# PreferredAI/PyBMF

Hardware: AMD Instinct MI355X
Metric: MU iterations/sec (BinaryMF-Penalty, 100k x 20k Boolean, k=64) (higher is better)
Workload: dtype i8 (bits x int8 digit planes on the integer MFMA, exact int32 accumulation); fp64 master factors and scalars; 1 GPU; BinaryMF-Penalty MU, 100000x20000 dense Boolean X, k=64, reg=1 growth=1.02, init normal+balance seed 2024; mae_pass=False, operands=i8x3, splits_xv=2, splits_xtu=11

## Files before the change

### include/bmf_hip.h

```cpp
#ifndef BMF_HIP_H
#define BMF_HIP_H

#include <stdint.h>

#ifdef __cplusplus
extern "C" {
#endif

#define BMF_OK 0
#define BMF_ERR_BAD_ARG (-1)
#define BMF_ERR_HIP (-2)
#define BMF_ERR_UNSUPPORTED (-3)
#define BMF_ERR_COMM (-4)

#define BMF_ROW_PAD 512
#define BMF_RED_PAD 128
#define BMF_MAX_KP 64
#define BMF_LOG_COLS 16

#define BMF_MODE_PREPARE 0
#define BMF_MODE_PENALTY 1
#define BMF_MODE_WNMF 2

enum {
// ... 146 lines not shown
int bmf_mae_sum_ex(const uint32_t* XTbits, int64_t ldxt, int64_t m_pad, int64_t n_pad, const float* U, const float* V, int kp,
                   uint16_t* ws, double* sum, int one_product, void* stream);
int bmf_mae_sum_tiled(const uint32_t* XTtiled, int64_t ldxt, int64_t m_pad, int64_t n_pad, const float* U, const float* V, int kp,
                      uint16_t* ws, double* sum, void* stream);

int bmf_mae_plan(int64_t m_pad, int64_t n_pad, int* groups, int* stages_per_group);


int bmf_cover_count(const uint32_t* Xbits, int64_t rows_pad, int64_t ldx, int64_t words, const uint64_t* rowbits,
                    const uint32_t* colbits, int64_t ldcb, int kp, unsigned long long* counts, const int32_t* stop,
                    void* stream);

int bmf_cover_delta(const uint32_t* bits, int64_t ld, int64_t words, int64_t rows_pad, const uint64_t* rowbits,
                    const uint64_t* rowbits_prev, const uint32_t* colbits, int64_t ldcb, int kp, unsigned long long* counts,
                    const uint64_t* copy_src, uint64_t* copy_dst, int64_t copy_n, const int32_t* stop, void* stream);

int bmf_confusion_rows(const uint32_t* Gbits, int64_t ldg, const uint32_t* Pbits, int64_t ldp, int64_t rows, int64_t words,
                       uint32_t* tp, uint32_t* fp, void* stream);

int bmf_boolean_product_bits(const uint64_t* rowbits, int64_t rows, const uint32_t* colbits, int64_t ldcb, int kp,
                             int64_t words, uint32_t* out, int64_t ldo, void* stream);

int bmf_real_product(const float* U, int64_t m_pad, int32_t m, const float* V, int64_t n_pad, int32_t n, int kp, float* out,
                     int64_t ldo, void* stream);


int bmf_residual_sums(const uint32_t* Xbits, int64_t m_pad, int64_t ldx, int32_t m, int32_t n, const float* U,
                      const float* V, int kp, double* sums, const int32_t* stop, void* stream);

int bmf_residual_plan(int64_t m, int64_t n, int* col_groups, int* tiles_per_group);
// ... 408 lines not shown
```

### pybmf_amd/_lib.py

```python
from __future__ import annotations

import ctypes as C
import os

import torch

_HERE = os.path.dirname(os.path.abspath(__file__))
LIB_PATH = os.path.join(_HERE, "csrc", os.environ.get("BMF_LIB", "libbmf_hip.so"))

BMF_OK = 0
ROW_PAD = 512
PANEL_BF16, PANEL_F16, PANEL_I8 = 0, 1, 2
LINK_SIGMOID, LINK_KL = 1, 2
PALM_ELBMF, PALM_PRIMP = 1, 2
NORM_SPECTRAL, NORM_FROBENIUS = 0, 1
RED_PAD = 128
MAX_KP = 64
LOG_COLS = 16
MODE_PREPARE, MODE_PENALTY, MODE_WNMF = 0, 1, 2
(LOG_ITER, LOG_ERROR, LOG_REC, LOG_REG, LOG_REGERR, LOG_RMSE, LOG_MAE, LOG_TP, LOG_FP, LOG_FN, LOG_TN, LOG_VALID,
 LOG_STOP) = range(13)

_vp, _i32, _i64, _f32, _f64 = C.c_void_p, C.c_int32, C.c_int64, C.c_float, C.c_double

# ... 137 lines not shown
    "bmf_mu_epilogue": (C.c_int, [C.POINTER(EpilogueArgs), _vp]),
    "bmf_masked_pass": (C.c_int, [_vp, _vp, _vp, _vp, _i32, _vp, _vp, _i32, _vp, _vp, _vp, C.c_int, _vp, _vp, _vp, _vp, _vp]),
    "bmf_masked_link_pass": (C.c_int, [_vp, _vp, _vp, _vp, _i32, _vp, _vp, _i32, _vp, _vp, _vp, C.c_int, _vp, _vp, _vp, _vp, C.c_int, _f64, _vp]),
    "bmf_masked_link_pass_k": (C.c_int, [_vp, _vp, _vp, _vp, _i32, _vp, _vp, _i32, _vp, _vp, _vp, C.c_int, C.c_int, _vp, _vp, _vp, _vp, C.c_int, _f64, _vp]),
    "bmf_masked_counts": (C.c_int, [_vp, _vp, _vp, _i64, _vp, _vp, _vp, _vp]),
    "bmf_masked_pass_wide": (C.c_int, [_vp, _vp, _vp, _vp, _i32, _vp, _vp, _i32, _vp] + [_vp] * 12),
    "bmf_masked_counts_wide": (C.c_int, [_vp, _vp, _vp, _i64, _vp, _vp, _vp, _vp, _vp, _vp]),
    "bmf_real_confusion": (C.c_int, [_vp, _i64, _i32, _i32, _vp, _vp, _vp, _vp]),
    "bmf_confusion_rows": (C.c_int, [_vp, _i64, _vp, _i64, _i64, _i64, _vp, _vp, _vp]),
    "bmf_mae_sum": (C.c_int, [_vp, _i64, _i64, _i64, _vp, _vp, C.c_int, _vp, _vp, _vp]),
    "bmf_mae_sum_ex": (C.c_int, [_vp, _i64, _i64, _i64, _vp, _vp, C.c_int, _vp, _vp, C.c_int, _vp]),
    "bmf_mae_sum_tiled": (C.c_int, [_vp, _i64, _i64, _i64, _vp, _vp, C.c_int, _vp, _vp, _vp]),
    "bmf_mae_plan": (C.c_int, [_i64, _i64, C.POINTER(C.c_int), C.POINTER(C.c_int)]),
    "bmf_cover_count": (C.c_int, [_vp, _i64, _i64, _i64, _vp, _vp, _i64, C.c_int, _vp, _vp, _vp]),
    "bmf_cover_delta": (C.c_int, [_vp, _i64, _i64, _i64, _vp, _vp, _vp, _i64, C.c_int, _vp, _vp, _vp, _i64, _vp, _vp]),
    "bmf_boolean_product_bits": (C.c_int, [_vp, _i64, _vp, _i64, C.c_int, _i64, _vp, _i64, _vp]),
    "bmf_real_product": (C.c_int, [_vp, _i64, _i32, _vp, _i64, _i32, C.c_int, _vp, _i64, _vp]),
    "bmf_residual_sums": (C.c_int, [_vp, _i64, _i64, _i32, _i32, _vp, _vp, C.c_int, _vp, _vp, _vp]),
    "bmf_residual_plan": (C.c_int, [_i64, _i64, C.POINTER(C.c_int), C.POINTER(C.c_int)]),
    "bmf_sqdiff_work": (_i64, []),
    "bmf_sqdiff_sum": (C.c_int, [_vp, _vp, _vp, _i64, _vp, _vp, _vp]),
    "bmf_residual_sums_f32": (C.c_int, [_vp, _i64, _i64, _i32, _i32, _vp, _vp, C.c_int, _vp, _vp]),
    "bmf_penalty_prepare": (C.c_int, [C.POINTER(PenaltyState), _vp]),
    "bmf_penalty_update": (C.c_int, [C.POINTER(PenaltyState), _f64, _vp]),
    "bmf_penalty_update_head": (C.c_int, [C.POINTER(PenaltyState), _f64, _vp]),
    "bmf_penalty_update_xtu": (C.c_int, [C.POINTER(PenaltyState), _i32, _vp]),
    "bmf_penalty_finalize": (C.c_int, [C.POINTER(PenaltyState), _i32, _f64, _i32, _vp]),
    "bmf_penalty_run": (C.c_int, [C.POINTER(PenaltyState), _i32, _i32, C.POINTER(_f64), _i32, _vp]),
    "bmf_comm_available": (C.c_int, []),
    "bmf_comm_unique_id": (C.c_int, [_vp]),
# ... 146 lines not shown
```

### pybmf_amd/csrc/api.hip

```cpp
#include "common.h"
#include "comm.h"

#include <cstdlib>
#include <vector>

int bmf_xf_bits_launch(const uint32_t* Abits, int64_t rows_pad, int64_t ldw, int64_t red_words, const uint16_t* panel,
                        int64_t ldp, int terms, int kp, float* out, int64_t slab_stride, int splits, int panel_kind,
                        const float* colscale, const int32_t* stop, hipStream_t s);
int bmf_mae_launch(const uint32_t* XTbits, int64_t ldxt, int64_t m_pad, int64_t n_pad, const float* U, const float* V, int kp,
                   uint16_t* ws, double* sum, const int32_t* stop, hipStream_t s, int one_product, int x_tiled, int zero_sums);
int bmf_panel_f16_launch(const float* F, int64_t rows_pad, int64_t ldf, int kp, uint16_t* panel, int64_t ldp, float* ws,
                         float* scale, bool have_blockmax, const int32_t* stop, hipStream_t s);
int bmf_panel_i8_launch(const double* F64, const float* F, int64_t rows_pad, int64_t ldf, int kp, int limbs, int8_t* panel, int64_t ldp,
                        float* ws, float* scale, bool have_blockmax, const int32_t* stop, hipStream_t s, bool have_scale,
                        const float* flags, float* colscale_out, const float* rslabs, int rcount, int rn, float* rout32, double* rout64);
int bmf_gram_partial_launch(const float* F, int64_t rows_pad, int64_t ldf, int kp, float* slabs, int blocks, const float* blockmax, int limbs,
                            float* scale, const int32_t* stop, hipStream_t s, int fused);
int bmf_xf_bits_i8_launch(const uint32_t* Abits, int64_t rows_pad, int64_t ldw, int64_t red_words, const int8_t* panel, int64_t ldp,
                          int limbs, const float* colscale, int kp, int col0, int ncols, float* out, int64_t slab_stride, int splits,
                          int a_tiled, const int32_t* stop, hipStream_t s);
int bmf_cover_launch(const uint32_t* Xbits, int64_t rows_pad, int64_t ldx, int64_t words, const uint64_t* rowbits,
                     const uint32_t* colbits, int64_t ldcb, int kp, unsigned long long* counts, const int32_t* stop,
                     hipStream_t s);
int bmf_cover_delta_launch(const uint32_t* bits, int64_t ld, int64_t words, int64_t rows_pad, const uint64_t* rowbits,
                           const uint64_t* rowbits_prev, const uint32_t* colbits, int64_t ldcb, int kp, unsigned long long* counts,
                           const uint64_t* copy_src, uint64_t* copy_dst, int64_t copy_n, const int32_t* stop, hipStream_t s);
int bmf_residual_launch(const uint32_t* Xbits, int64_t m_pad, int64_t ldx, int m, int n, const float* A, const float* B,
                        const float* dA, const float* dB, int kp, double* sums, const int32_t* stop, hipStream_t s);

namespace {
struct Timer {
    bool on = false, open = false;
    int cap = 0, used = 0, every = 1, seen = 0;
    std::vector<hipEvent_t> ev;
} g_timer;
}

void bmf_timer_begin(hipStream_t s) {
    g_timer.open = g_timer.on && g_timer.used < g_timer.cap && (g_timer.seen++ % g_timer.every) == 0;
    if (g_timer.open) (void)hipEventRecord(g_timer.ev[2 * g_timer.used], s);
}
// ... 267 lines not shown
        for (int sp = 0; sp < (stopped ? 0 : count); ++sp) acc += *reinterpret_cast<const f32x4*>(slabs + (int64_t)sp * slab_stride + row * kp + 32 * block + c4);
        *reinterpret_cast<f32x4*>(out + ((int64_t)block * rows_pad + row) * 32 + c4) = acc;
    }
}
}

static int xtu_slots_used(const bmf_penalty_state* st) {
    int n = st->splits_xtu;
    if (st->panel_kind == BMF_PANEL_I8) {
        const int need = bmf_xf_bits_i8_slots(st->n_pad, st->m_pad / 32, st->nred_blocks == 2 ? 32 : st->kp);
        if (need >= 1 && need < n) n = need;
    }
    return n;
}

enum { SWEEP_HEAD = 1, SWEEP_XTU = 2, SWEEP_SCALARS = 4, SWEEP_ALL = 7 };
static int sweep(const bmf_penalty_state* st, int mode, double reg, hipStream_t s, int phase = SWEEP_ALL, int block = -1, bool gather_in_finalize = false,
                 bool reduce_in_finalize = false) {
    const int kp = st->kp, kk = kp * kp;
    const int32_t* stop = st->stop;
    const bool f16 = st->panel_kind == BMF_PANEL_F16, i8 = st->panel_kind == BMF_PANEL_I8;
    const bool blocked = st->nred_blocks == 2;
    static const bool fused_planes = [] { const char* e = getenv("BMF_I8_FUSED_PLANES"); return !(e && e[0] == '0'); }();
    const int epi_terms = (f16 || i8) ? 0 : st->terms;
    const bool delta = st->ubits_prev && !st->updates_only;

    if (phase & SWEEP_HEAD) {
        bmf_epilogue_args ev = {};
        ev.F64 = st->V64; ev.F = st->V; ev.rows_pad = st->n_pad; ev.rows = st->n; ev.k = st->k; ev.kp = kp;
        ev.num = mode == BMF_MODE_PREPARE ? nullptr : st->Nred; ev.slab_stride = st->n_pad * kp; ev.splits = 1;
        ev.num_block_stride = blocked ? st->n_pad * 32 : 0;
        ev.G = st->GU; ev.reg = reg; ev.mode = mode; ev.thr = st->thr_v; ev.terms = epi_terms;
        ev.panel = st->Vpanel; ev.ldp = st->n_pad; ev.rowbits = st->vbits; ev.colbits = st->vcolbits; ev.ldcb = st->ldvc;
        ev.partials = st->partV; ev.stop = stop; ev.blockmax = (f16 || i8) ? st->panel_ws : nullptr;
        if (i8 && fused_planes) { ev.planes = (int8_t*)st->Vpanel; ev.plane_scale = st->scaleV; ev.limbs = st->terms; }
        BMF_TRY(bmf_mu_epilogue(&ev, s));
        if (f16) BMF_TRY(bmf_panel_f16_launch(st->V, st->n_pad, kp, kp, st->Vpanel, st->n_pad, st->panel_ws, st->scaleV, true, stop, s));
        BMF_TRY(bmf_gram_partial_launch(st->V, st->n_pad, kp, kp, st->gram_slabs, st->gram_blocks, i8 ? st->panel_ws : nullptr, st->terms, st->scaleV, stop, s, fused_planes ? 1 : 0));
        if (i8 && fused_planes)
            BMF_TRY(bmf_panel_i8_launch(st->V64, st->V, st->n_pad, kp, kp, st->terms, (int8_t*)st->Vpanel, st->n_pad, st->panel_ws, st->scaleV + 2 * kp, true, stop, s, true,
                                        st->scaleV + 3 * kp, st->scaleV + kp, st->gram_slabs, st->gram_blocks, kk, st->GV, st->GV64));
        else {
            if (i8)
                BMF_TRY(bmf_panel_i8_launch(st->V64, st->V, st->n_pad, kp, kp, st->terms, (int8_t*)st->Vpanel, st->n_pad, st->panel_ws, st->scaleV, true, stop, s, true, nullptr, nullptr,
                                            nullptr, 0, 0, nullptr, nullptr));
            BMF_TRY(bmf_reduce_slabs(st->gram_slabs, kk, st->gram_blocks, kk, st->GV, st->GV64, s));
        }
        if (delta && mode != BMF_MODE_PREPARE)
            BMF_TRY(bmf_cover_delta_launch(st->XTbits, st->ldxt, st->m_pad / 32, st->n_pad, st->vbits, st->vbits_prev, st->ucolbits, st->lduc, kp,
                                           st->counts, st->ubits, st->ubits_prev, st->m_pad, stop, s));

        bmf_timer_begin(s);
        if (i8)
            BMF_TRY(bmf_xf_bits_i8_launch(st->Xtiled ? st->Xtiled : st->Xbits, st->m_pad, st->ldx, st->n_pad / 32, (const int8_t*)st->Vpanel,
                                          st->n_pad, st->terms, st->scaleV + kp, kp, 0, kp, st->Mslab, st->m_pad * kp, st->splits_xv,
                                          st->Xtiled != nullptr, stop, s));
        else
            BMF_TRY(bmf_xf_bits_launch(st->Xbits, st->m_pad, st->ldx, st->n_pad / 32, st->Vpanel, st->n_pad, st->terms, kp, st->Mslab,
                                       st->m_pad * kp, st->splits_xv, st->panel_kind, f16 ? st->scaleV + kp : nullptr, stop, s));
        bmf_timer_end(s);

        bmf_epilogue_args eu = {};
        eu.F64 = st->U64; eu.F = st->U; eu.rows_pad = st->m_pad; eu.rows = st->m; eu.k = st->k; eu.kp = kp;
        const bool presum = st->splits_xv >= 6;
        if (presum)
            BMF_TRY(bmf_reduce_slabs(st->Mslab, st->m_pad * kp, st->splits_xv, st->m_pad * kp, st->Mslab, nullptr, s));
        eu.num = st->Mslab; eu.slab_stride = st->m_pad * kp; eu.splits = presum ? 1 : st->splits_xv;
        eu.G = st->GV; eu.reg = reg; eu.mode = mode; eu.thr = st->thr_u; eu.terms = epi_terms;
        eu.panel = st->Upanel; eu.ldp = st->m_pad; eu.rowbits = st->ubits; eu.colbits = st->ucolbits; eu.ldcb = st->lduc;
        eu.partials = st->partU; eu.stop = stop; eu.blockmax = (f16 || i8) ? st->panel_ws : nullptr;
        if (i8 && fused_planes) { eu.planes = (int8_t*)st->Upanel; eu.plane_scale = st->scaleU; eu.limbs = st->terms; }
        BMF_TRY(bmf_mu_epilogue(&eu, s));
        if (f16) BMF_TRY(bmf_panel_f16_launch(st->U, st->m_pad, kp, kp, st->Upanel, st->m_pad, st->panel_ws, st->scaleU, true, stop, s));
        BMF_TRY(bmf_gram_partial_launch(st->U, st->m_pad, kp, kp, st->gram_slabs, st->gram_blocks, i8 ? st->panel_ws : nullptr, st->terms, st->scaleU, stop, s, fused_planes ? 1 : 0));
        if (i8 && fused_planes)
            BMF_TRY(bmf_panel_i8_launch(st->U64, st->U, st->m_pad, kp, kp, st->terms, (int8_t*)st->Upanel, st->m_pad, st->panel_ws, st->scaleU + 2 * kp, true, stop, s, true,
                                        st->scaleU + 3 * kp, st->scaleU + kp, st->gram_slabs, st->gram_blocks, kk, nullptr, st->comm + 8));
        else {
            if (i8)
                BMF_TRY(bmf_panel_i8_launch(st->U64, st->U, st->m_pad, kp, kp, st->terms, (int8_t*)st->Upanel, st->m_pad, st->panel_ws, st->scaleU, true, stop, s, true, nullptr, nullptr,
                                            nullptr, 0, 0, nullptr, nullptr));
            BMF_TRY(bmf_reduce_slabs(st->gram_slabs, kk, st->gram_blocks, kk, nullptr, st->comm + 8, s));
        }
    }
    if (phase & SWEEP_SCALARS) {
        if (delta && mode != BMF_MODE_PREPARE) {
            BMF_TRY(bmf_cover_delta_launch(st->Xbits, st->ldx, st->n_pad / 32, st->m_pad, st->ubits, st->ubits_prev, st->vcolbits, st->ldvc, kp,
                                           st->counts, st->vbits, st->vbits_prev, st->n_pad, stop, s));
        } else if (!st->updates_only) {
            BMF_TRY(bmf_cover_launch(st->Xbits, st->m_pad, st->ldx, st->n_pad / 32, st->ubits, st->vcolbits, st->ldvc, kp, st->counts,
                                     stop, s));
            if (delta) {
                BMF_LAUNCH(rebase_cover_kernel, dim3(64), dim3(256), 0, s, st->ubits, st->ubits_prev, st->m_pad, st->vbits, st->vbits_prev, st->n_pad,
                           st->counts, stop);
                BMF_LAUNCH_CHECK();
            }
        }
        if (st->with_mae && !st->updates_only) {
            const bool one_product = st->m_pad * st->n_pad >= (1 << 24);
            if (!(st->mae_ws && one_product)) BMF_LAUNCH(zero_mae_kernel, dim3(1), dim3(64), 0, s, st->comm, stop);
            if (st->mae_ws) {
                const bool xt = st->XTtiled && st->m_pad * st->n_pad >= (1 << 24) && st->n_pad % 256 == 0 && st->ldxt % 16 == 0 && st->ldxt * 32 == st->m_pad;
                BMF_TRY(bmf_mae_launch(xt ? st->XTtiled : st->XTbits, st->ldxt, st->m_pad, st->n_pad, st->U, st->V, kp, st->mae_ws, st->comm + 4, stop, s,
// ... 96 lines not shown
}

static bool overlap_exchange(const bmf_penalty_state* st, const bmf_comm* c) {
    static const int env = [] { const char* e = getenv("BMF_EXCHANGE_OVERLAP"); return e ? (e[0] == '0' ? 0 : 1) : -1; }();
    if (env >= 0) return env == 1;
    if (c->world <= 1 || st->updates_only) return false;
    if (st->exchange_overlap != 0) return st->exchange_overlap == 2;
    return bmf_exchange_overlap_rule(st->with_mae, st->m_pad) != 0;
}

int exchange_phase(const bmf_penalty_state* st, bmf_comm* c, hipStream_t s) {
    const int kp = st->kp;
    const int64_t n32 = st->n_pad * kp, n64 = 8 + (int64_t)kp * kp;
    const bool timed = c->t_used < c->t_cap;
    const bool overlap = overlap_exchange(st, c);
    if (!overlap) BMF_TRY(sweep(st, st->mode, 0.0, s, SWEEP_SCALARS));
    if (timed) BMF_HIP_CHECK(hipEventRecord(c->tev[3 * c->t_used], s));
    if (st->nred_blocks == 2) {
        BMF_TRY(sweep(st, st->mode, 0.0, s, SWEEP_XTU, 0));
        BMF_TRY(fence_to_comm(c, 0, s));
        if (overlap) {
            BMF_TRY(bmf_comm_allreduce_on(c, st->Nred, n32 / 2, BMF_DTYPE_F32, c->cs));
        } else {
            BMF_TRY(bmf_comm_group_begin(c));
            int rc = bmf_comm_allreduce_on(c, st->Nred, n32 / 2, BMF_DTYPE_F32, c->cs);
            if (rc == BMF_OK) rc = bmf_comm_allreduce_on(c, st->comm, n64, BMF_DTYPE_F64, c->cs);
            const int rce = bmf_comm_group_end(c);
            if (rc != BMF_OK || rce != BMF_OK) return rc != BMF_OK ? rc : rce;
        }
        BMF_TRY(sweep(st, st->mode, 0.0, s, SWEEP_XTU, 1));
        BMF_TRY(fence_to_comm(c, 1, s));
// ... 64 lines not shown
    BMF_LAUNCH(finalize_kernel, dim3(1), dim3(1024), 0, s, *st, 0, reg0, (int)max_iter, 0);
    BMF_LAUNCH_CHECK();
    return BMF_OK;
}

extern "C" int bmf_penalty_run_sharded(const bmf_penalty_state* st, bmf_comm* comm, int32_t iter0, int32_t iter1, const double* regs_host,
                                       int32_t max_iter, void* stream) {
    BMF_TRY(check_state(st, "bmf_penalty_run_sharded"));
    BMF_TRY(check_comm(st, comm, "bmf_penalty_run_sharded"));
    BMF_REQUIRE(regs_host, "bmf_penalty_run_sharded: null regs_host");
    BMF_REQUIRE(iter0 >= 1 && iter1 >= iter0 && iter1 <= st->log_rows, "bmf_penalty_run_sharded: bad iteration range [%d,%d) for %d log rows",
                iter0, iter1, st->log_rows);
    hipStream_t s = (hipStream_t)stream;
    for (int it = iter0; it < iter1; ++it) {
        const double reg = regs_host[it - iter0];
        BMF_TRY(sweep(st, st->mode, reg, s, SWEEP_HEAD));
        BMF_TRY(exchange_phase(st, comm, s));
        BMF_LAUNCH(finalize_kernel, dim3(1), dim3(1024), 0, s, *st, it, reg, (int)max_iter, 0);
        BMF_LAUNCH_CHECK();
    }
    return BMF_OK;
}
```

### pybmf_amd/csrc/common.h

```cpp
#pragma once
#include <hip/hip_runtime.h>
#include <stdint.h>
#include <stdio.h>
#include <stdarg.h>

#include "../../include/bmf_hip.h"

typedef __attribute__((ext_vector_type(8))) __bf16 bf16x8;
typedef __attribute__((ext_vector_type(16))) float f32x16;
typedef __attribute__((ext_vector_type(4))) float f32x4;
typedef __attribute__((ext_vector_type(4))) unsigned u32x4;
typedef __attribute__((ext_vector_type(2))) unsigned u32x2;

#define BMF_EPS_F 2.220446049250313e-16f
#define BMF_EPS_D 2.220446049250313e-16

void bmf_set_error(const char* fmt, ...);
#define BMF_REQUIRE(cond, ...)                 \
    do {                                       \
        if (!(cond)) {                         \
            bmf_set_error(__VA_ARGS__);        \
            return BMF_ERR_BAD_ARG;            \
        }                                      \
    } while (0)
// ... 81 lines not shown
    }
    return t;
}
__device__ __forceinline__ double wave_sum(double v) {
#pragma unroll
    for (int o = 32; o > 0; o >>= 1) v += __shfl_xor(v, o, 64);
    return v;
}
__device__ __forceinline__ unsigned wave_sum(unsigned v) {
#pragma unroll
    for (int o = 32; o > 0; o >>= 1) v += __shfl_xor(v, o, 64);
    return v;
}

__device__ __forceinline__ void bmf_colscale_i8_block(const float* __restrict__ blockmax, int nblk, int kp, int limbs,
                                                      float* __restrict__ scale, int blk, float* sh) {
    const int cl = threadIdx.x & 3, sub = threadIdx.x >> 2;
    const int c = blk * 4 + cl;
    float m0 = 0.f;
    for (int b = sub; b < nblk; b += 64) m0 = fmaxf(m0, blockmax[(int64_t)b * kp + c]);
    sh[threadIdx.x] = m0;
    __syncthreads();
    for (int o = 128; o >= 4; o >>= 1) {
        if (threadIdx.x < o) sh[threadIdx.x] = fmaxf(sh[threadIdx.x], sh[threadIdx.x + o]);
        __syncthreads();
    }
    if (threadIdx.x < 4) {
        const float m = sh[threadIdx.x];
        int e = 0;
        if (m > 0.f && m <= 3.0e38f) {
            int ex;
            const float f = frexpf(m, &ex);
#ifdef BMF_EXP_QMAX_FRAC
            e = min(max((f > BMF_EXP_QMAX_FRAC ? BMF_EXP_QMAX_EXP - 1 : BMF_EXP_QMAX_EXP) - ex, -100), 100);
#else
            e = min(max((f > 0.99599f ? 22 : 23) - ex, -100), 100);
#endif
        }
        scale[c] = ldexpf(1.0f, e);
        scale[kp + c] = ldexpf(1.0f, (limbs == 2 ? 8 : 0) - e);
    }
}

__device__ __forceinline__ void bmf_colscale_i8_fused_block(const float* __restrict__ blockmax, int nblk, int kp, int limbs,
                                                            float* __restrict__ scale, int blk, float* sh) {
    const int cl = threadIdx.x & 3, sub = threadIdx.x >> 2;
    const int c = blk * 4 + cl;
    float m0 = 0.f;
    for (int b = sub; b < nblk; b += 64) m0 = fmaxf(m0, blockmax[(int64_t)b * kp + c]);
    sh[threadIdx.x] = m0;
    __syncthreads();
    for (int o = 128; o >= 4; o >>= 1) {
        if (threadIdx.x < o) sh[threadIdx.x] = fmaxf(sh[threadIdx.x], sh[threadIdx.x + o]);
        __syncthreads();
    }
    if (threadIdx.x < 4) {
        const float m = sh[threadIdx.x];
        int e = 0;
        if (m > 0.f && m <= 3.0e38f) {
            int ex;
            const float f = frexpf(m, &ex);
#ifdef BMF_EXP_QMAX_FRAC
            e = min(max((f > BMF_EXP_QMAX_FRAC ? BMF_EXP_QMAX_EXP - 1 : BMF_EXP_QMAX_EXP) - ex, -100), 100);
#else
            e = min(max((f > 0.99599f ? 22 : 23) - ex, -100), 100);
#endif
        }
        const float used = scale[c];
        const float v = m * used;
#ifdef BMF_EXP_QMAX_FRAC
        const bool ok = used > 0.f && used <= 3.0e38f && (m == 0.f || (v <= BMF_EXP_QMAX_FRAC * (float)(1 << BMF_EXP_QMAX_EXP) && v >= (float)(1 << (BMF_EXP_QMAX_EXP - 2))));
#else
        const bool ok = used > 0.f && used <= 3.0e38f && (m == 0.f || (v <= 8355711.0f && v >= 2097152.0f));
#endif
        const float fresh = ldexpf(1.0f, e);
        scale[kp + c] = (limbs == 2 ? 256.0f : 1.0f) / (ok ? used : fresh);
        scale[2 * kp + c] = fresh;
        scale[3 * kp + c] = ok ? 0.0f : 1.0f;
        scale[c] = fresh;
    }
}

__device__ __forceinline__ uint16_t bf16_bits(float x) {
    __bf16 b = (__bf16)x;
    return __builtin_bit_cast(uint16_t, b);
}
__device__ __forceinline__ float bf16_to_f32(uint16_t b) { return __uint_as_float(((unsigned)b) << 16); }

__device__ __forceinline__ void bmf_split3_bf16(const float (&x)[8], u32x4& hi, u32x4& mid, u32x4& lo) {
    unsigned xb[8], mb[8], lb[8];
#pragma unroll
    for (int j = 0; j < 8; ++j) {
        xb[j] = __float_as_uint(x[j]);
        const float r1 = x[j] - __uint_as_float(xb[j] & 0xffff0000u);
        mb[j] = __float_as_uint(r1);
        lb[j] = __float_as_uint(r1 - __uint_as_float(mb[j] & 0xffff0000u));
    }
// ... 11 lines not shown
```

### pybmf_amd/csrc/cover.hip

```cpp
#include "common.h"

#include <algorithm>
#include <cstdlib>

namespace {

constexpr int RB = 8, NW = 8;
constexpr int CH = 256;

__global__ __launch_bounds__(512) void cover_kernel(const uint32_t* __restrict__ X, int64_t ldx, int64_t words,
                                                     const uint64_t* __restrict__ rowbits,
                                                     const uint32_t* __restrict__ colbits, int64_t ldcb, int kp,
                                                     int64_t rows_pad, int rows_per_block, int y_big, int rows_big,
                                                     unsigned long long* __restrict__ counts,
                                                     const int32_t* __restrict__ stop) {
    if (stop && *stop != 0) return;
    __shared__ __attribute__((aligned(16))) uint32_t vt[BMF_MAX_KP + 1][CH];
    const int lane = threadIdx.x & 63;
    const int wave = __builtin_amdgcn_readfirstlane(threadIdx.x >> 6);
    const int64_t w0 = (int64_t)blockIdx.x * CH;
    const int nw = (int)min((int64_t)CH, words - w0);

    {
        constexpr int PIECES = BMF_MAX_KP * CH / 4;
// ... 224 lines not shown
    }
    tp = wave_sum(tp);
    pp = wave_sum(pp);
    __syncthreads();
    if (lane == 0) { vt[wave] = tp; vt[NWV + wave] = pp; }
    __syncthreads();
    if (threadIdx.x < 2) {
        unsigned long long t = 0, a_ = 0;
#pragma unroll
        for (int w = 0; w < NWV; ++w) { t += vt[w]; a_ += vt[NWV + w]; }
        const unsigned long long val = threadIdx.x == 0 ? t : a_ - t;
        if (val) atomicAdd(&counts[threadIdx.x], val);
    }
}

__global__ __launch_bounds__(1024) void cover_delta_kernel(const uint32_t* __restrict__ X, int64_t ldx, int64_t words, int chunk_words,
                                                            const uint64_t* __restrict__ rowbits, const uint64_t* __restrict__ rowbits_prev,
                                                            const uint32_t* __restrict__ colbits, int64_t ldcb, int kp, int64_t rows_pad,
                                                            int rows_per_block, unsigned long long* __restrict__ counts,
                                                            const uint64_t* __restrict__ copy_src, uint64_t* __restrict__ copy_dst, int64_t copy_n,
                                                            const int32_t* __restrict__ stop) {
    if (stop && *stop != 0) return;
    constexpr int CW = 640, NWV = 16, NS = 3;
    __shared__ __attribute__((aligned(16))) uint32_t vt[BMF_MAX_KP * CW];
    const int lane = threadIdx.x & 63;
    const int wave = __builtin_amdgcn_readfirstlane(threadIdx.x >> 6);
    const int64_t w0 = (int64_t)blockIdx.x * chunk_words;
    const int nw = (int)min((int64_t)chunk_words, words - w0);
    const int64_t r0 = (int64_t)blockIdx.y * rows_per_block;
    const int64_t r1 = min(r0 + rows_per_block, rows_pad);

    if (copy_n > 0) {
        const int64_t nthreads = (int64_t)gridDim.x * gridDim.y * 1024;
        for (int64_t i = ((int64_t)blockIdx.y * gridDim.x + blockIdx.x) * 1024 + threadIdx.x; i < copy_n; i += nthreads) copy_dst[i] = copy_src[i];
    }

    unsigned long long need = 0ull;
    for (int64_t r = r0 + threadIdx.x; r < r1; r += 1024) {
        const unsigned long long a_ = rowbits[r], b_ = rowbits_prev[r];
        if (a_ != b_) need |= a_ | b_;
    }
    if (threadIdx.x < 2) vt[threadIdx.x] = 0u;
    __syncthreads();
    if (need) {
        atomicOr(&vt[0], (unsigned)need);
        atomicOr(&vt[1], (unsigned)(need >> 32));
    }
    __syncthreads();
    need = ((unsigned long long)vt[1] << 32) | vt[0];
// ... 144 lines not shown
#pragma unroll
            for (int sg = 0; sg < NS; ++sg) x_cur[sg] = x_nxt[sg];
        }
    }
    int tp = (int)wave_sum(tpn - tpo);
    int pp = (int)wave_sum(ppn - ppo);
    __syncthreads();
    if (lane == 0) { vt[wave] = (unsigned)tp; vt[NWV + wave] = (unsigned)pp; }
    __syncthreads();
    if (threadIdx.x < 2) {
        long long t = 0, a_ = 0;
#pragma unroll
        for (int w = 0; w < NWV; ++w) { t += (int)vt[w]; a_ += (int)vt[NWV + w]; }
        const long long val = threadIdx.x == 0 ? t : a_ - t;
        if (val) atomicAdd(&counts[threadIdx.x], (unsigned long long)val);
    }
}

__global__ __launch_bounds__(256) void product_bits_kernel(const uint64_t* __restrict__ rowbits, int64_t rows,
                                                            const uint32_t* __restrict__ colbits, int64_t ldcb, int64_t words,
                                                            uint32_t* __restrict__ out, int64_t ldo) {
    const int64_t total = rows * words;
    for (int64_t idx = (int64_t)blockIdx.x * 256 + threadIdx.x; idx < total; idx += (int64_t)gridDim.x * 256) {
        const int64_t row = idx / words, w = idx - row * words;
        unsigned long long u = rowbits[row];
        unsigned pd = 0u;
        while (u) {
            const int l = __builtin_ctzll(u);
            u &= u - 1;
            pd |= colbits[(int64_t)l * ldcb + w];
// ... 96 lines not shown
}

extern "C" int bmf_cover_count(const uint32_t* Xbits, int64_t rows_pad, int64_t ldx, int64_t words,
                               const uint64_t* rowbits, const uint32_t* colbits, int64_t ldcb, int kp,
                               unsigned long long* counts, const int32_t* stop, void* stream) {
    BMF_REQUIRE(Xbits && rowbits && colbits && counts, "bmf_cover_count: null pointer");
    BMF_REQUIRE(rows_pad > 0 && rows_pad % 64 == 0, "bmf_cover_count: rows_pad must be a positive multiple of 64");
    BMF_REQUIRE(words > 0 && words % 4 == 0 && ldx >= words && ldx % 4 == 0, "bmf_cover_count: words/ldx must be multiples of 4, ldx >= words");
    BMF_REQUIRE(ldcb >= words && ldcb % 4 == 0, "bmf_cover_count: ldcb must be >= words and a multiple of 4");
    BMF_REQUIRE(bmf_aligned16(colbits), "bmf_cover_count: colbits must be 16-byte aligned");
    BMF_REQUIRE(kp >= 1 && kp <= BMF_MAX_KP, "bmf_cover_count: kp must be 1..64");
    BMF_REQUIRE(bmf_aligned16(Xbits), "bmf_cover_count: Xbits must be 16-byte aligned");
    return bmf_cover_launch(Xbits, rows_pad, ldx, words, rowbits, colbits, ldcb, kp, counts, stop, (hipStream_t)stream);
}

int bmf_cover_delta_launch(const uint32_t* bits, int64_t ld, int64_t words, int64_t rows_pad, const uint64_t* rowbits,
                           const uint64_t* rowbits_prev, const uint32_t* colbits, int64_t ldcb, int kp, unsigned long long* counts,
                           const uint64_t* copy_src, uint64_t* copy_dst, int64_t copy_n, const int32_t* stop, hipStream_t s) {
    const int chunks_w = (int)((words + 639) / 640);
    const int64_t per = (words + chunks_w - 1) / chunks_w;
    const int cw = (int)(words >= 128 ? (per + 127) / 128 * 128 : words);
    const int cus = bmf_cu_count_current();
    int64_t groups = cus / chunks_w > 0 ? cus / chunks_w : 1;
    const int64_t units = rows_pad / 64;
    if (groups > units) groups = units;
    const int rows_per_block = (int)(((units + groups - 1) / groups) * 64);
    groups = (rows_pad + rows_per_block - 1) / rows_per_block;
    BMF_LAUNCH(cover_delta_kernel, dim3((unsigned)chunks_w, (unsigned)groups), dim3(1024), 0, s, bits, ld, words, cw, rowbits, rowbits_prev, colbits,
               ldcb, kp, rows_pad, rows_per_block, counts, copy_src, copy_dst, copy_n, stop);
    BMF_LAUNCH_CHECK();
    return BMF_OK;
}

extern "C" int bmf_cover_delta(const uint32_t* bits, int64_t ld, int64_t words, int64_t rows_pad, const uint64_t* rowbits,
                               const uint64_t* rowbits_prev, const uint32_t* colbits, int64_t ldcb, int kp, unsigned long long* counts,
                               const uint64_t* copy_src, uint64_t* copy_dst, int64_t copy_n, const int32_t* stop, void* stream) {
    BMF_REQUIRE(bits && rowbits && rowbits_prev && colbits && counts, "bmf_cover_delta: null pointer");
    BMF_REQUIRE(rows_pad > 0 && rows_pad % 64 == 0, "bmf_cover_delta: rows_pad must be a positive multiple of 64");
    BMF_REQUIRE(words >= 4 && words % 4 == 0 && ld >= words && ld % 4 == 0, "bmf_cover_delta: words/ld must be multiples of 4, ld >= words >= 4");
    BMF_REQUIRE(ldcb >= words && ldcb % 4 == 0, "bmf_cover_delta: ldcb must be >= words and a multiple of 4");
    BMF_REQUIRE(bmf_aligned16(bits) && bmf_aligned16(colbits), "bmf_cover_delta: bits and colbits must be 16-byte aligned");
    BMF_REQUIRE(kp >= 1 && kp <= BMF_MAX_KP, "bmf_cover_delta: kp must be 1..64");
    BMF_REQUIRE(copy_n >= 0 && (copy_n == 0 || (copy_src && copy_dst)), "bmf_cover_delta: copy_n > 0 needs copy_src and copy_dst");
    BMF_REQUIRE(copy_n == 0 || (copy_dst != rowbits && copy_dst != rowbits_prev), "bmf_cover_delta: the copy must not overwrite the words this launch compares");
    return bmf_cover_delta_launch(bits, ld, words, rows_pad, rowbits, rowbits_prev, colbits, ldcb, kp, counts, copy_src, copy_dst, copy_n, stop,
                                  (hipStream_t)stream);
// ... 14 lines not shown
```

Baseline: 1941 iterations/s.

## Merge Gram partial and cover-delta kernels into one role-split launch

Adds a combined kernel in which some workgroups run the cover-delta bit counting, others compute the Gram partial slabs, and a few compute the i8 column scales, all in a single launch. The sweep uses it in place of separate Gram and cover-delta launches for the V side, and also for the U side when the scalar phase runs with the head. This moves the row cover-delta out of the scalar phase. The aim is to save launches and let the two independent workloads share the GPU at the same time. The cost is larger per-block LDS and register use and workgroups that serialize cover-delta then Gram work, which may lengthen the critical path.

```diff
diff --git a/include/bmf_hip.h b/include/bmf_hip.h
--- a/include/bmf_hip.h
+++ b/include/bmf_hip.h
@@ -184,6 +184,12 @@
 int bmf_cover_delta(const uint32_t* bits, int64_t ld, int64_t words, int64_t rows_pad, const uint64_t* rowbits,
                     const uint64_t* rowbits_prev, const uint32_t* colbits, int64_t ldcb, int kp, unsigned long long* counts,
                     const uint64_t* copy_src, uint64_t* copy_dst, int64_t copy_n, const int32_t* stop, void* stream);
+
+int bmf_gram_cover_delta(const float* F, int64_t rows_pad, int64_t ldf, int kp, float* slabs, int blocks, const float* blockmax, int limbs,
+                         float* scale, int fused, const uint32_t* bits, int64_t ld, int64_t words, int64_t bit_rows_pad,
+                         const uint64_t* rowbits, const uint64_t* rowbits_prev, const uint32_t* colbits, int64_t ldcb,
+                         unsigned long long* counts, const uint64_t* copy_src, uint64_t* copy_dst, int64_t copy_n, const int32_t* stop,
+                         void* stream);
 
 int bmf_confusion_rows(const uint32_t* Gbits, int64_t ldg, const uint32_t* Pbits, int64_t ldp, int64_t rows, int64_t words,
                        uint32_t* tp, uint32_t* fp, void* stream);
diff --git a/pybmf_amd/_lib.py b/pybmf_amd/_lib.py
--- a/pybmf_amd/_lib.py
+++ b/pybmf_amd/_lib.py
@@ -175,6 +175,8 @@
     "bmf_mae_plan": (C.c_int, [_i64, _i64, C.POINTER(C.c_int), C.POINTER(C.c_int)]),
     "bmf_cover_count": (C.c_int, [_vp, _i64, _i64, _i64, _vp, _vp, _i64, C.c_int, _vp, _vp, _vp]),
     "bmf_cover_delta": (C.c_int, [_vp, _i64, _i64, _i64, _vp, _vp, _vp, _i64, C.c_int, _vp, _vp, _vp, _i64, _vp, _vp]),
+    "bmf_gram_cover_delta": (C.c_int, [_vp, _i64, _i64, C.c_int, _vp, C.c_int, _vp, C.c_int, _vp, C.c_int,
+                                       _vp, _i64, _i64, _i64, _vp, _vp, _vp, _i64, _vp, _vp, _vp, _i64, _vp, _vp]),
     "bmf_boolean_product_bits": (C.c_int, [_vp, _i64, _vp, _i64, C.c_int, _i64, _vp, _i64, _vp]),
     "bmf_real_product": (C.c_int, [_vp, _i64, _i32, _vp, _i64, _i32, C.c_int, _vp, _i64, _vp]),
     "bmf_residual_sums": (C.c_int, [_vp, _i64, _i64, _i32, _i32, _vp, _vp, C.c_int, _vp, _vp, _vp]),
diff --git a/pybmf_amd/csrc/api.hip b/pybmf_amd/csrc/api.hip
--- a/pybmf_amd/csrc/api.hip
+++ b/pybmf_amd/csrc/api.hip
@@ -25,6 +25,10 @@
 int bmf_cover_delta_launch(const uint32_t* bits, int64_t ld, int64_t words, int64_t rows_pad, const uint64_t* rowbits,
                            const uint64_t* rowbits_prev, const uint32_t* colbits, int64_t ldcb, int kp, unsigned long long* counts,
                            const uint64_t* copy_src, uint64_t* copy_dst, int64_t copy_n, const int32_t* stop, hipStream_t s);
+int bmf_gram_cover_delta_launch(const float* F, int64_t rows_pad, int64_t ldf, int kp, float* slabs, int blocks, const float* blockmax, int limbs,
+                                float* scale, int fused, const uint32_t* bits, int64_t ld, int64_t words, int64_t bit_rows_pad, const uint64_t* rowbits,
+                                const uint64_t* rowbits_prev, const uint32_t* colbits, int64_t ldcb, unsigned long long* counts,
+                                const uint64_t* copy_src, uint64_t* copy_dst, int64_t copy_n, const int32_t* stop, hipStream_t s);
 int bmf_residual_launch(const uint32_t* Xbits, int64_t m_pad, int64_t ldx, int m, int n, const float* A, const float* B,
                         const float* dA, const float* dB, int kp, double* sums, const int32_t* stop, hipStream_t s);
 
@@ -322,7 +326,7 @@
     return n;
 }
 
-enum { SWEEP_HEAD = 1, SWEEP_XTU = 2, SWEEP_SCALARS = 4, SWEEP_ALL = 7 };
+enum { SWEEP_HEAD = 1, SWEEP_XTU = 2, SWEEP_SCALARS = 4, SWEEP_ALL = 7, SWEEP_ROW_IN_HEAD = 8 };
 static int sweep(const bmf_penalty_state* st, int mode, double reg, hipStream_t s, int phase = SWEEP_ALL, int block = -1, bool gather_in_finalize = false,
                  bool reduce_in_finalize = false) {
     const int kp = st->kp, kk = kp * kp;
@@ -332,6 +336,8 @@
     static const bool fused_planes = [] { const char* e = getenv("BMF_I8_FUSED_PLANES"); return !(e && e[0] == '0'); }();
     const int epi_terms = (f16 || i8) ? 0 : st->terms;
     const bool delta = st->ubits_prev && !st->updates_only;
+    const bool merged = delta && mode != BMF_MODE_PREPARE;
+    const bool row_in_head = merged && ((phase & SWEEP_ROW_IN_HEAD) || ((phase & SWEEP_HEAD) && (phase & SWEEP_SCALARS)));
 
     if (phase & SWEEP_HEAD) {
         bmf_epilogue_args ev = {};
@@ -344,7 +350,12 @@
         if (i8 && fused_planes) { ev.planes = (int8_t*)st->Vpanel; ev.plane_scale = st->scaleV; ev.limbs = st->terms; }
         BMF_TRY(bmf_mu_epilogue(&ev, s));
         if (f16) BMF_TRY(bmf_panel_f16_launch(st->V, st->n_pad, kp, kp, st->Vpanel, st->n_pad, st->panel_ws, st->scaleV, true, stop, s));
-        BMF_TRY(bmf_gram_partial_launch(st->V, st->n_pad, kp, kp, st->gram_slabs, st->gram_blocks, i8 ? st->panel_ws : nullptr, st->terms, st->scaleV, stop, s, fused_planes ? 1 : 0));
+        if (merged)
+            BMF_TRY(bmf_gram_cover_delta_launch(st->V, st->n_pad, kp, kp, st->gram_slabs, st->gram_blocks, i8 ? st->panel_ws : nullptr, st->terms, st->scaleV,
+                                                fused_planes ? 1 : 0, st->XTbits, st->ldxt, st->m_pad / 32, st->n_pad, st->vbits, st->vbits_prev, st->ucolbits,
+                                                st->lduc, st->counts, st->ubits, st->ubits_prev, st->m_pad, stop, s));
+        else
+            BMF_TRY(bmf_gram_partial_launch(st->V, st->n_pad, kp, kp, st->gram_slabs, st->gram_blocks, i8 ? st->panel_ws : nullptr, st->terms, st->scaleV, stop, s, fused_planes ? 1 : 0));
         if (i8 && fused_planes)
             BMF_TRY(bmf_panel_i8_launch(st->V64, st->V, st->n_pad, kp, kp, st->terms, (int8_t*)st->Vpanel, st->n_pad, st->panel_ws, st->scaleV + 2 * kp, true, stop, s, true,
                                         st->scaleV + 3 * kp, st->scaleV + kp, st->gram_slabs, st->gram_blocks, kk, st->GV, st->GV64));
@@ -354,10 +365,6 @@
                                             nullptr, 0, 0, nullptr, nullptr));
             BMF_TRY(bmf_reduce_slabs(st->gram_slabs, kk, st->gram_blocks, kk, st->GV, st->GV64, s));
         }
-        if (delta && mode != BMF_MODE_PREPARE)
-            BMF_TRY(bmf_cover_delta_launch(st->XTbits, st->ldxt, st->m_pad / 32, st->n_pad, st->vbits, st->vbits_prev, st->ucolbits, st->lduc, kp,
-                                           st->counts, st->ubits, st->ubits_prev, st->m_pad, stop, s));
-
         bmf_timer_begin(s);
         if (i8)
             BMF_TRY(bmf_xf_bits_i8_launch(st->Xtiled ? st->Xtiled : st->Xbits, st->m_pad, st->ldx, st->n_pad / 32, (const int8_t*)st->Vpanel,
@@ -380,7 +387,12 @@
         if (i8 && fused_planes) { eu.planes = (int8_t*)st->Upanel; eu.plane_scale = st->scaleU; eu.limbs = st->terms; }
         BMF_TRY(bmf_mu_epilogue(&eu, s));
         if (f16) BMF_TRY(bmf_panel_f16_launch(st->U, st->m_pad, kp, kp, st->Upanel, st->m_pad, st->panel_ws, st->scaleU, true, stop, s));
-        BMF_TRY(bmf_gram_partial_launch(st->U, st->m_pad, kp, kp, st->gram_slabs, st->gram_blocks, i8 ? st->panel_ws : nullptr, st->terms, st->scaleU, stop, s, fused_planes ? 1 : 0));
+        if (row_in_head)
+            BMF_TRY(bmf_gram_cover_delta_launch(st->U, st->m_pad, kp, kp, st->gram_slabs, st->gram_blocks, i8 ? st->panel_ws : nullptr, st->terms, st->scaleU,
+                                                fused_planes ? 1 : 0, st->Xbits, st->ldx, st->n_pad / 32, st->m_pad, st->ubits, st->ubits_prev, st->vcolbits,
+                                                st->ldvc, st->counts, st->vbits, st->vbits_prev, st->n_pad, stop, s));
+        else
+            BMF_TRY(bmf_gram_partial_launch(st->U, st->m_pad, kp, kp, st->gram_slabs, st->gram_blocks, i8 ? st->panel_ws : nullptr, st->terms, st->scaleU, stop, s, fused_planes ? 1 : 0));
         if (i8 && fused_planes)
             BMF_TRY(bmf_panel_i8_launch(st->U64, st->U, st->m_pad, kp, kp, st->terms, (int8_t*)st->Upanel, st->m_pad, st->panel_ws, st->scaleU + 2 * kp, true, stop, s, true,
                                         st->scaleU + 3 * kp, st->scaleU + kp, st->gram_slabs, st->gram_blocks, kk, nullptr, st->comm + 8));
@@ -393,8 +405,9 @@
     }
     if (phase & SWEEP_SCALARS) {
         if (delta && mode != BMF_MODE_PREPARE) {
-            BMF_TRY(bmf_cover_delta_launch(st->Xbits, st->ldx, st->n_pad / 32, st->m_pad, st->ubits, st->ubits_prev, st->vcolbits, st->ldvc, kp,
-                                           st->counts, st->vbits, st->vbits_prev, st->n_pad, stop, s));
+            if (!row_in_head)
+                BMF_TRY(bmf_cover_delta_launch(st->Xbits, st->ldx, st->n_pad / 32, st->m_pad, st->ubits, st->ubits_prev, st->vcolbits, st->ldvc, kp,
+                                               st->counts, st->vbits, st->vbits_prev, st->n_pad, stop, s));
         } else if (!st->updates_only) {
             BMF_TRY(bmf_cover_launch(st->Xbits, st->m_pad, st->ldx, st->n_pad / 32, st->ubits, st->vcolbits, st->ldvc, kp, st->counts,
                                      stop, s));
@@ -521,7 +534,7 @@
     const int64_t n32 = st->n_pad * kp, n64 = 8 + (int64_t)kp * kp;
     const bool timed = c->t_used < c->t_cap;
     const bool overlap = overlap_exchange(st, c);
-    if (!overlap) BMF_TRY(sweep(st, st->mode, 0.0, s, SWEEP_SCALARS));
+    if (!overlap) BMF_TRY(sweep(st, st->mode, 0.0, s, SWEEP_SCALARS | SWEEP_ROW_IN_HEAD));
     if (timed) BMF_HIP_CHECK(hipEventRecord(c->tev[3 * c->t_used], s));
     if (st->nred_blocks == 2) {
         BMF_TRY(sweep(st, st->mode, 0.0, s, SWEEP_XTU, 0));
@@ -616,7 +629,7 @@
     hipStream_t s = (hipStream_t)stream;
     for (int it = iter0; it < iter1; ++it) {
         const double reg = regs_host[it - iter0];
-        BMF_TRY(sweep(st, st->mode, reg, s, SWEEP_HEAD));
+        BMF_TRY(sweep(st, st->mode, reg, s, SWEEP_HEAD | (overlap_exchange(st, comm) ? 0 : SWEEP_ROW_IN_HEAD)));
         BMF_TRY(exchange_phase(st, comm, s));
         BMF_LAUNCH(finalize_kernel, dim3(1), dim3(1024), 0, s, *st, it, reg, (int)max_iter, 0);
         BMF_LAUNCH_CHECK();
diff --git a/pybmf_amd/csrc/common.h b/pybmf_amd/csrc/common.h
--- a/pybmf_amd/csrc/common.h
+++ b/pybmf_amd/csrc/common.h
@@ -119,19 +119,20 @@
 }
 
 __device__ __forceinline__ void bmf_colscale_i8_block(const float* __restrict__ blockmax, int nblk, int kp, int limbs,
-                                                      float* __restrict__ scale, int blk, float* sh) {
-    const int cl = threadIdx.x & 3, sub = threadIdx.x >> 2;
+                                                      float* __restrict__ scale, int blk, float* sh, int tid, bool on) {
+    const int cl = tid & 3, sub = tid >> 2;
     const int c = blk * 4 + cl;
     float m0 = 0.f;
-    for (int b = sub; b < nblk; b += 64) m0 = fmaxf(m0, blockmax[(int64_t)b * kp + c]);
-    sh[threadIdx.x] = m0;
+    if (on)
+        for (int b = sub; b < nblk; b += 64) m0 = fmaxf(m0, blockmax[(int64_t)b * kp + c]);
+    sh[tid] = m0;
     __syncthreads();
     for (int o = 128; o >= 4; o >>= 1) {
-        if (threadIdx.x < o) sh[threadIdx.x] = fmaxf(sh[threadIdx.x], sh[threadIdx.x + o]);
+        if (tid < o) sh[tid] = fmaxf(sh[tid], sh[tid + o]);
         __syncthreads();
     }
-    if (threadIdx.x < 4) {
-        const float m = sh[threadIdx.x];
+    if (on && tid < 4) {
+        const float m = sh[tid];
         int e = 0;
         if (m > 0.f && m <= 3.0e38f) {
             int ex;
@@ -148,19 +149,20 @@
 }
 
 __device__ __forceinline__ void bmf_colscale_i8_fused_block(const float* __restrict__ blockmax, int nblk, int kp, int limbs,
-                                                            float* __restrict__ scale, int blk, float* sh) {
-    const int cl = threadIdx.x & 3, sub = threadIdx.x >> 2;
+                                                            float* __restrict__ scale, int blk, float* sh, int tid, bool on) {
+    const int cl = tid & 3, sub = tid >> 2;
     const int c = blk * 4 + cl;
     float m0 = 0.f;
-    for (int b = sub; b < nblk; b += 64) m0 = fmaxf(m0, blockmax[(int64_t)b * kp + c]);
-    sh[threadIdx.x] = m0;
+    if (on)
+        for (int b = sub; b < nblk; b += 64) m0 = fmaxf(m0, blockmax[(int64_t)b * kp + c]);
+    sh[tid] = m0;
     __syncthreads();
     for (int o = 128; o >= 4; o >>= 1) {
-        if (threadIdx.x < o) sh[threadIdx.x] = fmaxf(sh[threadIdx.x], sh[threadIdx.x + o]);
+        if (tid < o) sh[tid] = fmaxf(sh[tid], sh[tid + o]);
         __syncthreads();
     }
-    if (threadIdx.x < 4) {
-        const float m = sh[threadIdx.x];
+    if (on && tid < 4) {
+        const float m = sh[tid];
         int e = 0;
         if (m > 0.f && m <= 3.0e38f) {
             int ex;
@@ -186,6 +188,15 @@
     }
 }
 
+__device__ __forceinline__ void bmf_colscale_i8_block(const float* __restrict__ blockmax, int nblk, int kp, int limbs,
+                                                      float* __restrict__ scale, int blk, float* sh) {
+    bmf_colscale_i8_block(blockmax, nblk, kp, limbs, scale, blk, sh, (int)threadIdx.x, true);
+}
+__device__ __forceinline__ void bmf_colscale_i8_fused_block(const float* __restrict__ blockmax, int nblk, int kp, int limbs,
+                                                            float* __restrict__ scale, int blk, float* sh) {
+    bmf_colscale_i8_fused_block(blockmax, nblk, kp, limbs, scale, blk, sh, (int)threadIdx.x, true);
+}
+
 __device__ __forceinline__ uint16_t bf16_bits(float x) {
     __bf16 b = (__bf16)x;
     return __builtin_bit_cast(uint16_t, b);
diff --git a/pybmf_amd/csrc/cover.hip b/pybmf_amd/csrc/cover.hip
--- a/pybmf_amd/csrc/cover.hip
+++ b/pybmf_amd/csrc/cover.hip
@@ -262,25 +262,23 @@
     }
 }
 
-__global__ __launch_bounds__(1024) void cover_delta_kernel(const uint32_t* __restrict__ X, int64_t ldx, int64_t words, int chunk_words,
-                                                            const uint64_t* __restrict__ rowbits, const uint64_t* __restrict__ rowbits_prev,
-                                                            const uint32_t* __restrict__ colbits, int64_t ldcb, int kp, int64_t rows_pad,
-                                                            int rows_per_block, unsigned long long* __restrict__ counts,
-                                                            const uint64_t* __restrict__ copy_src, uint64_t* __restrict__ copy_dst, int64_t copy_n,
-                                                            const int32_t* __restrict__ stop) {
-    if (stop && *stop != 0) return;
-    constexpr int CW = 640, NWV = 16, NS = 3;
-    __shared__ __attribute__((aligned(16))) uint32_t vt[BMF_MAX_KP * CW];
+constexpr int CD_CW = 640;
+__device__ __forceinline__ void cover_delta_block(uint32_t* vt, int bx, int by, int nbx, int nby, const uint32_t* __restrict__ X, int64_t ldx,
+                                                  int64_t words, int chunk_words, const uint64_t* __restrict__ rowbits,
+                                                  const uint64_t* __restrict__ rowbits_prev, const uint32_t* __restrict__ colbits, int64_t ldcb,
+                                                  int kp, int64_t rows_pad, int rows_per_block, unsigned long long* __restrict__ counts,
+                                                  const uint64_t* __restrict__ copy_src, uint64_t* __restrict__ copy_dst, int64_t copy_n) {
+    constexpr int CW = CD_CW, NWV = 16, NS = 3;
     const int lane = threadIdx.x & 63;
     const int wave = __builtin_amdgcn_readfirstlane(threadIdx.x >> 6);
-    const int64_t w0 = (int64_t)blockIdx.x * chunk_words;
+    const int64_t w0 = (int64_t)bx * chunk_words;
     const int nw = (int)min((int64_t)chunk_words, words - w0);
-    const int64_t r0 = (int64_t)blockIdx.y * rows_per_block;
+    const int64_t r0 = (int64_t)by * rows_per_block;
     const int64_t r1 = min(r0 + rows_per_block, rows_pad);
 
     if (copy_n > 0) {
-        const int64_t nthreads = (int64_t)gridDim.x * gridDim.y * 1024;
-        for (int64_t i = ((int64_t)blockIdx.y * gridDim.x + blockIdx.x) * 1024 + threadIdx.x; i < copy_n; i += nthreads) copy_dst[i] = copy_src[i];
+        const int64_t nthreads = (int64_t)nbx * nby * 1024;
+        for (int64_t i = ((int64_t)by * nbx + bx) * 1024 + threadIdx.x; i < copy_n; i += nthreads) copy_dst[i] = copy_src[i];
     }
 
     unsigned long long need = 0ull;
@@ -455,6 +453,100 @@
         for (int w = 0; w < NWV; ++w) { t += (int)vt[w]; a_ += (int)vt[NWV + w]; }
         const long long val = threadIdx.x == 0 ? t : a_ - t;
         if (val) atomicAdd(&counts[threadIdx.x], (unsigned long long)val);
+    }
+}
+
+struct cover_delta_args {
+    const uint32_t* X; int64_t ldx, words; int chunk_words;
+    const uint64_t* rowbits; const uint64_t* rowbits_prev; const uint32_t* colbits; int64_t ldcb; int kp; int64_t rows_pad; int rows_per_block;
+    unsigned long long* counts; const uint64_t* copy_src; uint64_t* copy_dst; int64_t copy_n;
+};
+
+__global__ __launch_bounds__(1024) void cover_delta_kernel(cover_delta_args c, const int32_t* __restrict__ stop) {
+    if (stop && *stop != 0) return;
+    __shared__ __attribute__((aligned(16))) uint32_t vt[BMF_MAX_KP * CD_CW];
+    cover_delta_block(vt, (int)blockIdx.x, (int)blockIdx.y, (int)gridDim.x, (int)gridDim.y, c.X, c.ldx, c.words, c.chunk_words, c.rowbits, c.rowbits_prev,
+                      c.colbits, c.ldcb, c.kp, c.rows_pad, c.rows_per_block, c.counts, c.copy_src, c.copy_dst, c.copy_n);
+}
+
+struct gram_role_args {
+    const float* F; int64_t rows_pad, ldf; float* slabs; int gram_blocks; const float* blockmax; int nblk, limbs; float* scale; int fused;
+};
+
+template <int A, int B>
+__device__ __forceinline__ void bmf_gram_wave_tile(const float* __restrict__ F, int64_t ldf, int64_t p0, int64_t p1, int lane, f32x16& acc) {
+    const int c = lane & 31, h = lane >> 5;
+    const float* fp = F + (2 * p0 + h) * ldf + c;
+    int64_t p = p0;
+    for (; p + 8 <= p1; p += 8) {
+        float va[8], vb[8];
+#pragma unroll
+        for (int u = 0; u < 8; ++u) {
+            va[u] = fp[(int64_t)(2 * u) * ldf + 32 * A];
+            vb[u] = A == B ? va[u] : fp[(int64_t)(2 * u) * ldf + 32 * B];
+        }
+        fp += 16 * ldf;
+#pragma unroll
+        for (int u = 0; u < 8; ++u) acc = __builtin_amdgcn_mfma_f32_32x32x2f32(va[u], vb[u], acc, 0, 0, 0);
+    }
+    for (; p < p1; ++p) {
+        const float va = fp[32 * A], vb = A == B ? va : fp[32 * B];
+        fp += 2 * ldf;
+        acc = __builtin_amdgcn_mfma_f32_32x32x2f32(va, vb, acc, 0, 0, 0);
+    }
+}
+
+template <int NT>
+__global__ __launch_bounds__(1024) void gram_cover_delta_kernel(gram_role_args g, cover_delta_args c, int gram_wgs, int scale_wgs, int nbx, int nby,
+                                                                 const int32_t* __restrict__ stop) {
+    constexpr int KP = 32 * NT, NTILES = NT * (NT + 1) / 2;
+    constexpr int QF = BMF_MAX_KP * CD_CW / 4;
+    static_assert(NT == 1 || NT == 2, "tiles are numbered a + b");
+    static_assert(NTILES * 4 * 1024 <= 4 * QF && QF >= 256, "the partial tiles must fit the LDS");
+    __shared__ __attribute__((aligned(16))) uint32_t vt[BMF_MAX_KP * CD_CW];
+    const int bid = (int)blockIdx.x, ncover = nbx * nby;
+    float* lds = reinterpret_cast<float*>(vt);
+    if (bid >= max(ncover, gram_wgs)) {
+        if (stop && *stop != 0) return;
+        const int q = __builtin_amdgcn_readfirstlane((int)threadIdx.x >> 8), tid = (int)threadIdx.x & 255;
+        const int blk = (bid - max(ncover, gram_wgs)) * 4 + q;
+        const bool on = blk < KP / 4;
+        if (g.fused) bmf_colscale_i8_fused_block(g.blockmax, g.nblk, KP, g.limbs, g.scale, blk, lds + q * QF, tid, on);
+        else bmf_colscale_i8_block(g.blockmax, g.nblk, KP, g.limbs, g.scale, blk, lds + q * QF, tid, on);
+        return;
+    }
+    if (bid < ncover && !(stop && *stop != 0)) {
+        cover_delta_block(vt, bid % nbx, bid / nbx, nbx, nby, c.X, c.ldx, c.words, c.chunk_words, c.rowbits, c.rowbits_prev, c.colbits, c.ldcb, c.kp,
+                          c.rows_pad, c.rows_per_block, c.counts, c.copy_src, c.copy_dst, c.copy_n);
+        __syncthreads();
+    }
+    if (bid >= gram_wgs) return;
+    const int lane = (int)threadIdx.x & 63, wv = __builtin_amdgcn_readfirstlane((int)threadIdx.x >> 6);
+    const int t = wv >> 2, w = wv & 3;
+    if (t < NTILES) {
+        const int64_t nwaves = (int64_t)g.gram_blocks * 4;
+        const int64_t gw = (int64_t)bid * 4 + w;
+        const int64_t pairs = g.rows_pad / 2;
+        const int64_t per = (pairs + nwaves - 1) / nwaves;
+        const int64_t p0 = gw * per, p1 = min(p0 + per, pairs);
+        f32x16 acc;
+#pragma unroll
+        for (int i = 0; i < 16; ++i) acc[i] = 0.f;
+        if (t == 0) bmf_gram_wave_tile<0, 0>(g.F, g.ldf, p0, p1, lane, acc);
+        else if (t == 1) bmf_gram_wave_tile<0, NT - 1>(g.F, g.ldf, p0, p1, lane, acc);
+        else bmf_gram_wave_tile<NT - 1, NT - 1>(g.F, g.ldf, p0, p1, lane, acc);
+        float* slot = lds + wv * 1024 + lane;
+#pragma unroll
+        for (int i = 0; i < 16; ++i) slot[i * 64] = acc[i];
+    }
+    __syncthreads();
+    float* o = g.slabs + (int64_t)bid * KP * KP;
+    for (int e = (int)threadIdx.x; e < KP * KP; e += 1024) {
+        int r = e / KP, cc = e % KP;
+        if ((cc >> 5) < (r >> 5)) { const int x = r; r = cc; cc = x; }
+        const int tile = (r >> 5) + (cc >> 5), rr = r & 31;
+        const float* s_ = lds + tile * 4096 + ((rr & 3) + 4 * (rr >> 3)) * 64 + 32 * ((rr >> 2) & 1) + (cc & 31);
+        o[e] = (s_[0] + s_[1024]) + (s_[2048] + s_[3072]);
     }
 }
 
@@ -581,22 +673,66 @@
     return bmf_cover_launch(Xbits, rows_pad, ldx, words, rowbits, colbits, ldcb, kp, counts, stop, (hipStream_t)stream);
 }
 
+static void cover_delta_plan(cover_delta_args* c, int* chunks_w_out, int* groups_out) {
+    const int chunks_w = (int)((c->words + 639) / 640);
+    const int64_t per = (c->words + chunks_w - 1) / chunks_w;
+    c->chunk_words = (int)(c->words >= 128 ? (per + 127) / 128 * 128 : c->words);
+    const int cus = bmf_cu_count_current();
+    int64_t groups = cus / chunks_w > 0 ? cus / chunks_w : 1;
+    const int64_t units = c->rows_pad / 64;
+    if (groups > units) groups = units;
+    c->rows_per_block = (int)(((units + groups - 1) / groups) * 64);
+    *chunks_w_out = chunks_w;
+    *groups_out = (int)((c->rows_pad + c->rows_per_block - 1) / c->rows_per_block);
+}
+
 int bmf_cover_delta_launch(const uint32_t* bits, int64_t ld, int64_t words, int64_t rows_pad, const uint64_t* rowbits,
                            const uint64_t* rowbits_prev, const uint32_t* colbits, int64_t ldcb, int kp, unsigned long long* counts,
                            const uint64_t* copy_src, uint64_t* copy_dst, int64_t copy_n, const int32_t* stop, hipStream_t s) {
-    const int chunks_w = (int)((words + 639) / 640);
-    const int64_t per = (words + chunks_w - 1) / chunks_w;
-    const int cw = (int)(words >= 128 ? (per + 127) / 128 * 128 : words);
-    const int cus = bmf_cu_count_current();
-    int64_t groups = cus / chunks_w > 0 ? cus / chunks_w : 1;
-    const int64_t units = rows_pad / 64;
-    if (groups > units) groups = units;
-    const int rows_per_block = (int)(((units + groups - 1) / groups) * 64);
-    groups = (rows_pad + rows_per_block - 1) / rows_per_block;
-    BMF_LAUNCH(cover_delta_kernel, dim3((unsigned)chunks_w, (unsigned)groups), dim3(1024), 0, s, bits, ld, words, cw, rowbits, rowbits_prev, colbits,
-               ldcb, kp, rows_pad, rows_per_block, counts, copy_src, copy_dst, copy_n, stop);
+    cover_delta_args c = {bits, ld, words, 0, rowbits, rowbits_prev, colbits, ldcb, kp, rows_pad, 0, counts, copy_src, copy_dst, copy_n};
+    int chunks_w, groups;
+    cover_delta_plan(&c, &chunks_w, &groups);
+    BMF_LAUNCH(cover_delta_kernel, dim3((unsigned)chunks_w, (unsigned)groups), dim3(1024), 0, s, c, stop);
     BMF_LAUNCH_CHECK();
     return BMF_OK;
+}
+
+int bmf_gram_cover_delta_launch(const float* F, int64_t rows_pad, int64_t ldf, int kp, float* slabs, int blocks, const float* blockmax, int limbs,
+                                float* scale, int fused, const uint32_t* bits, int64_t ld, int64_t words, int64_t bit_rows_pad, const uint64_t* rowbits,
+                                const uint64_t* rowbits_prev, const uint32_t* colbits, int64_t ldcb, unsigned long long* counts,
+                                const uint64_t* copy_src, uint64_t* copy_dst, int64_t copy_n, const int32_t* stop, hipStream_t s) {
+    gram_role_args g = {F, rows_pad, ldf, slabs, blocks, blockmax, (int)(rows_pad / 128), limbs, scale, fused};
+    cover_delta_args c = {bits, ld, words, 0, rowbits, rowbits_prev, colbits, ldcb, kp, bit_rows_pad, 0, counts, copy_src, copy_dst, copy_n};
+    int chunks_w, groups;
+    cover_delta_plan(&c, &chunks_w, &groups);
+    const int gram_wgs = blocks, scale_wgs = blockmax ? (kp / 4 + 3) / 4 : 0;
+    const dim3 grid((unsigned)(std::max(gram_wgs, chunks_w * groups) + scale_wgs));
+    if (kp == 32) BMF_LAUNCH(gram_cover_delta_kernel<1>, grid, dim3(1024), 0, s, g, c, gram_wgs, scale_wgs, chunks_w, groups, stop);
+    else BMF_LAUNCH(gram_cover_delta_kernel<2>, grid, dim3(1024), 0, s, g, c, gram_wgs, scale_wgs, chunks_w, groups, stop);
+    BMF_LAUNCH_CHECK();
+    return BMF_OK;
+}
+
+extern "C" int bmf_gram_cover_delta(const float* F, int64_t rows_pad, int64_t ldf, int kp, float* slabs, int blocks, const float* blockmax, int limbs,
+                                    float* scale, int fused, const uint32_t* bits, int64_t ld, int64_t words, int64_t bit_rows_pad,
+                                    const uint64_t* rowbits, const uint64_t* rowbits_prev, const uint32_t* colbits, int64_t ldcb,
+                                    unsigned long long* counts, const uint64_t* copy_src, uint64_t* copy_dst, int64_t copy_n, const int32_t* stop,
+                                    void* stream) {
+    BMF_REQUIRE(F && slabs, "bmf_gram_cover_delta: null pointer");
+    BMF_REQUIRE(rows_pad > 0 && rows_pad % 2 == 0, "bmf_gram_cover_delta: rows_pad must be even");
+    BMF_REQUIRE((kp == 32 || kp == 64) && ldf >= kp, "bmf_gram_cover_delta: kp must be 32 or 64 and ldf >= kp");
+    BMF_REQUIRE(blocks >= 1 && blocks <= 1024, "bmf_gram_cover_delta: blocks must be 1..1024");
+    BMF_REQUIRE(!blockmax || (scale && rows_pad % 128 == 0 && (limbs == 2 || limbs == 3)), "bmf_gram_cover_delta: bad column-scale arguments");
+    BMF_REQUIRE(fused == 0 || fused == 1, "bmf_gram_cover_delta: fused=%d must be 0 or 1", fused);
+    BMF_REQUIRE(bits && rowbits && rowbits_prev && colbits && counts, "bmf_gram_cover_delta: null pointer");
+    BMF_REQUIRE(bit_rows_pad > 0 && bit_rows_pad % 64 == 0, "bmf_gram_cover_delta: bit_rows_pad must be a positive multiple of 64");
+    BMF_REQUIRE(words >= 4 && words % 4 == 0 && ld >= words && ld % 4 == 0, "bmf_gram_cover_delta: words/ld must be multiples of 4, ld >= words >= 4");
+    BMF_REQUIRE(ldcb >= words && ldcb % 4 == 0, "bmf_gram_cover_delta: ldcb must be >= words and a multiple of 4");
+    BMF_REQUIRE(bmf_aligned16(bits) && bmf_aligned16(colbits), "bmf_gram_cover_delta: bits and colbits must be 16-byte aligned");
+    BMF_REQUIRE(copy_n >= 0 && (copy_n == 0 || (copy_src && copy_dst)), "bmf_gram_cover_delta: copy_n > 0 needs copy_src and copy_dst");
+    BMF_REQUIRE(copy_n == 0 || (copy_dst != rowbits && copy_dst != rowbits_prev), "bmf_gram_cover_delta: the copy must not overwrite the words this launch compares");
+    return bmf_gram_cover_delta_launch(F, rows_pad, ldf, kp, slabs, blocks, blockmax, limbs, scale, fused, bits, ld, words, bit_rows_pad, rowbits,
+                                       rowbits_prev, colbits, ldcb, counts, copy_src, copy_dst, copy_n, stop, (hipStream_t)stream);
 }
 
 extern "C" int bmf_cover_delta(const uint32_t* bits, int64_t ld, int64_t words, int64_t rows_pad, const uint64_t* rowbits,
```

Result: no change. 1934 iterations/s (-0.3%).
